# Zelana-Labs/zelana

Hardware: AMD Instinct MI355X
Metric: BN254 G1 MSM Mpoint-scalar/s + L2 proofs/sec at 1/2/4/8 MI355X (higher is better)
Workload: dtype u32

## Files before the change

### include/zkmi.h

```cpp
#ifndef ZKMI_H
#define ZKMI_H
#include <stddef.h>
#include <stdint.h>

#ifdef __cplusplus
extern "C" {
#endif

#define ZKMI_OK 0
#define ZKMI_EINVAL (-1)
#define ZKMI_ENODEV (-2)
#define ZKMI_EHIP (-3)
#define ZKMI_ENOMEM (-4)
#define ZKMI_EPOINT (-5)

typedef struct zkmi_ctx zkmi_ctx;
typedef struct zkmi_bases zkmi_bases;
typedef struct zkmi_pk zkmi_pk;
typedef struct zkmi_msm_job zkmi_msm_job;
typedef struct zkmi_r1cs_dev zkmi_r1cs_dev;

const char* zkmi_last_error(void);
int zkmi_version(void);

int zkmi_ctx_create(int device, zkmi_ctx** out);
void zkmi_ctx_destroy(zkmi_ctx* ctx);
int zkmi_profile_enable(zkmi_ctx* ctx, int on);
int zkmi_profile_get(zkmi_ctx* ctx, const char* name, double* total_ms, uint64_t* count);
int zkmi_profile_reset(zkmi_ctx* ctx);
int zkmi_dev_alloc(zkmi_ctx* ctx, size_t bytes, void** dptr);
int zkmi_dev_free(zkmi_ctx* ctx, void* dptr);
int zkmi_h2d(zkmi_ctx* ctx, void* dst, const void* src, size_t bytes);
int zkmi_d2h(zkmi_ctx* ctx, void* dst, const void* src, size_t bytes);
int zkmi_sync(zkmi_ctx* ctx);

int zkmi_bases_create_g1(zkmi_ctx* ctx, const uint64_t* affine, size_t n, zkmi_bases** out);
int zkmi_bases_create_g2(zkmi_ctx* ctx, const uint64_t* affine, size_t n, zkmi_bases** out);
void zkmi_bases_destroy(zkmi_bases* b);
size_t zkmi_bases_len(const zkmi_bases* b);
int zkmi_bases_export(const zkmi_bases* b, uint64_t* affine_out);
int zkmi_bases_precompute(zkmi_bases* b, int c, int factor);
int zkmi_bases_info(const zkmi_bases* b, uint64_t out[4]);
int zkmi_bases_generate_g1(zkmi_ctx* ctx, uint64_t seed, size_t n, zkmi_bases** out);
int zkmi_bases_generate_g2(zkmi_ctx* ctx, uint64_t seed, size_t n, zkmi_bases** out);
int zkmi_scalars_generate(zkmi_ctx* ctx, uint64_t seed, size_t n, void* d_scalars);
int zkmi_bases_generate_range_g1(zkmi_ctx* ctx, uint64_t seed, size_t first, size_t n, zkmi_bases** out);
int zkmi_scalars_generate_range(zkmi_ctx* ctx, uint64_t seed, size_t first, size_t n, void* d_scalars);
int zkmi_bases_generate_arith_g1(zkmi_ctx* ctx, const uint64_t p0[8], const uint64_t d[8], size_t first, size_t n,
                                 zkmi_bases** out);

int zkmi_msm_g1(zkmi_ctx* ctx, const zkmi_bases* b, size_t offset, const uint64_t* scalars, size_t n,
                uint64_t out_affine[8]);
int zkmi_msm_g2(zkmi_ctx* ctx, const zkmi_bases* b, size_t offset, const uint64_t* scalars, size_t n,
                uint64_t out_affine[16]);
int zkmi_msm_g1_device(zkmi_ctx* ctx, const zkmi_bases* b, size_t offset, const void* d_scalars, size_t n,
                       uint64_t out_affine[8]);
int zkmi_msm_g2_device(zkmi_ctx* ctx, const zkmi_bases* b, size_t offset, const void* d_scalars, size_t n,
                       uint64_t out_affine[16]);
int zkmi_msm_submit(zkmi_ctx* ctx, const zkmi_bases* b, size_t offset, const void* d_scalars, size_t n,
                    zkmi_msm_job** job);
int zkmi_msm_wait(zkmi_msm_job* job, uint64_t* out_affine);
int zkmi_msm_submit_shared(zkmi_ctx* ctx, const zkmi_bases* const* bs, int k, size_t offset, const void* d_scalars,
// ... 202 lines not shown
```

### zelana_amd/_lib.py

```python
from __future__ import annotations

import ctypes
import os

HERE = os.path.dirname(os.path.abspath(__file__))
LIB_PATH = os.environ.get("ZKMI_LIB") or os.path.join(HERE, "libzkmi.so")


class ZkmiError(RuntimeError):
    pass


_lib = None
vp = ctypes.c_void_p
u64p = ctypes.POINTER(ctypes.c_uint64)
u8p = ctypes.POINTER(ctypes.c_uint8)
sz = ctypes.c_size_t


class WprogDesc(ctypes.Structure):
    _fields_ = [
        ("num_vars", sz), ("num_inputs", sz), ("input_var", vp), ("num_ops", sz), ("op", vp),
        ("num_terms", sz), ("term", vp), ("num_coeffs", sz), ("coeff", vp), ("num_levels", sz),
        ("level_start", vp),
    ]


class R1CSStruct(ctypes.Structure):
    _fields_ = [
        ("num_constraints", sz), ("num_instance", sz), ("num_witness", sz),
        ("a_rowptr", vp), ("a_col", vp), ("a_val", vp),
        ("b_rowptr", vp), ("b_col", vp), ("b_val", vp),
        ("c_rowptr", vp), ("c_col", vp), ("c_val", vp),
    ]


class R1CSStatusStruct(ctypes.Structure):
    _fields_ = [("first_row", ctypes.c_uint64), ("n_bad", ctypes.c_uint64), ("a", ctypes.c_uint64 * 4),
                ("b", ctypes.c_uint64 * 4), ("c", ctypes.c_uint64 * 4)]


ROW_NONE = 2**64 - 1


class VerifyStatsStruct(ctypes.Structure):
    _fields_ = [("pairs", ctypes.c_uint64), ("final_exps", ctypes.c_uint64), ("invalid_points", ctypes.c_uint64)]


SIGNATURES = [
    ("zkmi_last_error", ctypes.c_char_p, []),
    ("zkmi_version", ctypes.c_int, []),
    ("zkmi_ctx_create", ctypes.c_int, [ctypes.c_int, ctypes.POINTER(vp)]),
    ("zkmi_ctx_destroy", None, [vp]),
    ("zkmi_profile_enable", ctypes.c_int, [vp, ctypes.c_int]),
    ("zkmi_profile_get", ctypes.c_int, [vp, ctypes.c_char_p, ctypes.POINTER(ctypes.c_double),
                                        ctypes.POINTER(ctypes.c_uint64)]),
    ("zkmi_profile_reset", ctypes.c_int, [vp]),
    ("zkmi_dev_alloc", ctypes.c_int, [vp, sz, ctypes.POINTER(vp)]),
    ("zkmi_dev_free", ctypes.c_int, [vp, vp]),
    ("zkmi_h2d", ctypes.c_int, [vp, vp, vp, sz]),
    ("zkmi_d2h", ctypes.c_int, [vp, vp, vp, sz]),
    ("zkmi_sync", ctypes.c_int, [vp]),
    ("zkmi_bases_create_g1", ctypes.c_int, [vp, u64p, sz, ctypes.POINTER(vp)]),
    ("zkmi_bases_create_g2", ctypes.c_int, [vp, u64p, sz, ctypes.POINTER(vp)]),
    ("zkmi_bases_destroy", None, [vp]),
    ("zkmi_bases_len", sz, [vp]),
    ("zkmi_bases_export", ctypes.c_int, [vp, u64p]),
    ("zkmi_bases_precompute", ctypes.c_int, [vp, ctypes.c_int, ctypes.c_int]),
    ("zkmi_bases_info", ctypes.c_int, [vp, u64p]),
    ("zkmi_bases_generate_g1", ctypes.c_int, [vp, ctypes.c_uint64, sz, ctypes.POINTER(vp)]),
    ("zkmi_bases_generate_g2", ctypes.c_int, [vp, ctypes.c_uint64, sz, ctypes.POINTER(vp)]),
    ("zkmi_scalars_generate", ctypes.c_int, [vp, ctypes.c_uint64, sz, vp]),
    ("zkmi_bases_generate_range_g1", ctypes.c_int, [vp, ctypes.c_uint64, sz, sz, ctypes.POINTER(vp)]),
    ("zkmi_bases_generate_arith_g1", ctypes.c_int, [vp, u64p, u64p, sz, sz, ctypes.POINTER(vp)]),
    ("zkmi_scalars_generate_range", ctypes.c_int, [vp, ctypes.c_uint64, sz, sz, vp]),
    ("zkmi_msm_g1", ctypes.c_int, [vp, vp, sz, u64p, sz, u64p]),
    ("zkmi_msm_g2", ctypes.c_int, [vp, vp, sz, u64p, sz, u64p]),
    ("zkmi_msm_g1_device", ctypes.c_int, [vp, vp, sz, vp, sz, u64p]),
    ("zkmi_msm_g2_device", ctypes.c_int, [vp, vp, sz, vp, sz, u64p]),
    ("zkmi_msm_submit", ctypes.c_int, [vp, vp, sz, vp, sz, ctypes.POINTER(vp)]),
    ("zkmi_msm_wait", ctypes.c_int, [vp, u64p]),
    ("zkmi_msm_set_window", ctypes.c_int, [vp, ctypes.c_int]),
    ("zkmi_msm_batch_submit", ctypes.c_int, [vp, vp, sz, vp, sz, sz, sz, ctypes.POINTER(vp)]),
    ("zkmi_msm_batch_wait", ctypes.c_int, [vp, u64p, sz]),
    ("zkmi_ctx_set_batch_group", ctypes.c_int, [vp, ctypes.c_int]),
    ("zkmi_ctx_get_batch_group", ctypes.c_int, [vp]),
    ("zkmi_msm_set_lanes", ctypes.c_int, [vp, ctypes.c_int]),
    ("zkmi_msm_get_lanes", ctypes.c_int, [vp]),
    ("zkmi_ctx_stream_count", ctypes.c_int, [vp]),
    ("zkmi_msm_submit_shared", ctypes.c_int, [vp, ctypes.POINTER(vp), ctypes.c_int, sz, vp, sz, ctypes.POINTER(vp)]),
# ... 129 lines not shown
```

### zelana_amd/csrc/ec.h

```cpp
#pragma once
#include "ff.h"

#if defined(__HIPCC__) || defined(__HIP__)
#define ZK_HD_NOINLINE __host__ __device__ __noinline__
#else
#define ZK_HD_NOINLINE inline
#endif

namespace zk {


template <class F>
struct Aff {
  typename F::T x, y;
};
template <class F>
struct Xyzz {
  typename F::T x, y, zz, zzz;
};

template <class F>
ZK_HD Xyzz<F> xyzz_inf() {
  Xyzz<F> r;
  r.x = F::zero();
// ... 93 lines not shown
  Fe qx = subk<FqP, 8>(qq, r.x);
  r.y = mul2<FqP>(rr, qx, ny1, ppp);
  r.zz = mul<FqP>(p.zz, pp);
  r.zzz = mul<FqP>(p.zzz, ppp);
  return r;
}
ZK_HD Xyzz<FqOps> xyzz_madd_g1f(const Xyzz<FqOps>& p, const Fe& qx, const Fe& qy, bool* inf) {
  const Fe ny1 = bsub(FqP::B4_1, p.y);
  const Fe pp_ = mul_add<FqP>(qx, p.zz, bsub(FqP::B8_1, p.x));
  const Fe rr = mul_add<FqP>(qy, p.zzz, ny1);
  const Fe pp = sqr<FqP>(pp_);
  uint32_t z = 0, e = 0;
#pragma unroll
  for (int i = 0; i < NL; i++) {
    z |= pp.v[i];
    e |= pp.v[i] ^ FqP::P[i];
  }
  *inf = false;
  if (z == 0 || e == 0) {
    if (is_zero<FqP>(reduce_q32<FqP>(rr))) return xyzz_mdbl(Aff<FqOps>{qx, reduce_q32<FqP>(qy)});
    *inf = true;
    return xyzz_inf<FqOps>();
  }
  const Fe ppp = mul<FqP>(pp_, pp);
  const Fe qq = mul<FqP>(p.x, pp);
  Xyzz<FqOps> r;
  r.x = sqr_add<FqP>(rr, bsub2(FqP::B6_3, ppp, qq));
  r.y = mul2<FqP>(rr, bsubadd(FqP::B10_1, r.x, qq), ny1, ppp);
  r.zz = mul<FqP>(p.zz, pp);
  r.zzz = mul<FqP>(p.zzz, ppp);
  return r;
}

ZK_HD Xyzz<FqOps> xyzz_mmadd_g1(const Aff<FqOps>& p, const Aff<FqOps>& q) {
  Fe pp_ = subk<FqP, 2>(q.x, p.x);
  Fe ny1 = subk<FqP, 2>(fe_zero(), p.y);
  Fe rr = add_lazy(q.y, ny1);
  Fe pp = sqr<FqP>(pp_);
  if (is_zero<FqP>(pp)) {
    Fe rn = reduce8<FqP>(subk<FqP, 2>(q.y, p.y));
    if (is_zero<FqP>(rn)) return xyzz_mdbl(q);
    return xyzz_inf<FqOps>();
  }
  Fe ppp = mul<FqP>(pp_, pp);
  Fe qq = mul<FqP>(p.x, pp);
  Fe t = add_lazy(add_lazy(ppp, qq), qq);
  Xyzz<FqOps> r;
  r.x = subk<FqP, 6>(sqr<FqP>(rr), t);
  Fe qx = subk<FqP, 8>(qq, r.x);
  r.y = mul2<FqP>(rr, qx, ny1, ppp);
  r.zz = pp;
  r.zzz = ppp;
  return r;
}
ZK_HD Xyzz<Fq2Ops> xyzz_mmadd_g2(const Aff<Fq2Ops>& p, const Aff<Fq2Ops>& q) {
  Fe2 pp_ = {subk<FqPn, 2>(q.x.c0, p.x.c0), subk<FqPn, 2>(q.x.c1, p.x.c1)};
  Fe2 rr = {subk<FqPn, 2>(q.y.c0, p.y.c0), subk<FqPn, 2>(q.y.c1, p.y.c1)};
  Fe2 pp = f2_sqr_n(pp_);
  if (f2_is_zero(pp)) {
    if (is_zero<FqPn>(reduce8<FqPn>(rr.c0)) && is_zero<FqPn>(reduce8<FqPn>(rr.c1))) return xyzz_mdbl(q);
    return xyzz_inf<Fq2Ops>();
  }
  Fe2 r2 = f2_sqr_n(rr);
  Fe2 ppp = f2_mul_n(pp_, pp), qq = f2_mul_n(p.x, pp);
  Xyzz<Fq2Ops> r;
  r.x.c0 = reduce8<FqPn>(subk<FqPn, 6>(r2.c0, add_lazy(add_lazy(ppp.c0, qq.c0), qq.c0)));
  r.x.c1 = reduce8<FqPn>(subk<FqPn, 6>(r2.c1, add_lazy(add_lazy(ppp.c1, qq.c1), qq.c1)));
  Fe2 qx = {subk<FqPn, 2>(qq.c0, r.x.c0), subk<FqPn, 2>(qq.c1, r.x.c1)};
  Fe ny0 = subk<FqPn, 2>(fe_zero(), p.y.c0), ny1 = subk<FqPn, 2>(fe_zero(), p.y.c1);
  Fe nqx1 = subk<FqPn, 4>(fe_zero(), qx.c1), nppp1 = subk<FqPn, 2>(fe_zero(), ppp.c1);
  r.y.c0 = mul4<FqPn>(rr.c0, qx.c0, rr.c1, nqx1, ny0, ppp.c0, ny1, nppp1);
  r.y.c1 = mul4<FqPn>(rr.c0, qx.c1, rr.c1, qx.c0, ny0, ppp.c1, ny1, ppp.c0);
  r.zz = pp;
  r.zzz = ppp;
  return r;
}
// ... 125 lines not shown
```

### zelana_amd/csrc/msm.hip

```cpp
#include <stdarg.h>
#include <stdlib.h>
#include <stdio.h>
#include <string.h>

#include <algorithm>
#include <string>
#include <type_traits>
#include <utility>
#include <vector>
#include <chrono>

#include "dev_io.h"
#include "ec.h"
#include "zkmi_internal.h"

namespace zk {

#define ZK_TAIL_WAVE() __builtin_amdgcn_s_setprio(3)

struct G1T {
  using F = FqOps;
  using P = FqP;
  static constexpr int CW = 8;
  static constexpr int PW = 16;
// ... 1059 lines not shown
#define ZK_ACC0_G2_MINBLK 2
#endif
#ifndef ZK_ACC0_G1_MINBLK
#define ZK_ACC0_G1_MINBLK 1
#endif
__global__ void __launch_bounds__(256, ZK_ACC0_G1_MINBLK) k_msm_acc0_g1(const uint32_t* __restrict__ sval, const uint32_t* __restrict__ bstart,
                                                  uint32_t K, uint32_t L, uint32_t nchunks,
                                                  const uint32_t* __restrict__ bases, uint32_t tn, uint32_t tskip,
                                                  uint32_t* __restrict__ buckets,
                                                  uint32_t* __restrict__ xkey, uint32_t* __restrict__ xvalid,
                                                  uint32_t* __restrict__ xpts, uint32_t* __restrict__ flags) { msm_acc0_body<G1T>(sval, bstart, K, L, nchunks, bases, tn, tskip, buckets, xkey, xvalid, xpts, flags); }
__global__ void __launch_bounds__(256, ZK_ACC0_G2_MINBLK) k_msm_acc0_g2(const uint32_t* __restrict__ sval, const uint32_t* __restrict__ bstart,
                                                  uint32_t K, uint32_t L, uint32_t nchunks,
                                                  const uint32_t* __restrict__ bases, uint32_t tn, uint32_t tskip,
                                                  uint32_t* __restrict__ buckets,
                                                  uint32_t* __restrict__ xkey, uint32_t* __restrict__ xvalid,
                                                  uint32_t* __restrict__ xpts, uint32_t* __restrict__ flags) { msm_acc0_body<G2T>(sval, bstart, K, L, nchunks, bases, tn, tskip, buckets, xkey, xvalid, xpts, flags); }
template <class G>
struct Acc0Kernel;
template <>
struct Acc0Kernel<G1T> {
  static constexpr auto fn = k_msm_acc0_g1;
};
template <>
struct Acc0Kernel<G2T> {
  static constexpr auto fn = k_msm_acc0_g2;
};

constexpr uint32_t ITEM_CAP_MAX = 1024;
constexpr uint32_t ITEMS_MIN_K = 1u << 18;
constexpr uint32_t NOSLOT = 0xFFFFFFFFu;

__device__ __forceinline__ bool item_of(const uint4* __restrict__ items, uint32_t nover, uint32_t nmain, uint32_t i,
                                        uint4& it) {
  uint32_t idx;
  if (i < nover) {
    idx = nmain + i;
  } else {
    idx = i - nover;
    if (idx >= nmain) return false;
  }
  it = items[idx];
  return it.x != it.y;
}

template <class G>
__device__ __forceinline__ void acc_items_body(const uint4* __restrict__ items, const uint32_t* __restrict__ nover,
                                               uint32_t nmain, const uint32_t* __restrict__ sval,
                                               const uint32_t* __restrict__ bases, uint32_t tn, uint32_t tskip,
                                               uint32_t* __restrict__ buckets, uint32_t* __restrict__ xpts) {
  using F = typename G::F;
  constexpr int XW = 4 * G::CW;
  constexpr int PQ = G::PW / 4;
  uint4 it;
  if (!item_of(items, *nover, nmain, blockIdx.x * blockDim.x + threadIdx.x, it)) return;
  const uint32_t start = it.x, end = it.y;
  auto row = [&](uint32_t v) {
    uint32_t idx = v & 0x7FFFFFFFu;
    if (tskip) idx += (idx / tn) * tskip;
    const uint32_t* src = bases;
    return reinterpret_cast<const uint4*>(src + (size_t)idx * G::PW);
  };
  constexpr bool PF = G::CW == 8;
  Xyzz<F> acc = xyzz_inf<F>();
  bool naff = false;
  uint32_t v_nxt = sval[start];
  uint4 raw[PQ];
  if constexpr (PF) {
    const uint4* q = row(v_nxt);
#pragma unroll
    for (int k = 0; k < PQ; k++) raw[k] = q[k];
  }
  uint32_t v_nn = start + 1 < end ? sval[start + 1] : 0u;
  for (uint32_t p = start; p < end; p++) {
    uint4 cr[PQ];
    const uint32_t v = v_nxt;
    if constexpr (PF) {
#pragma unroll
      for (int k = 0; k < PQ; k++) cr[k] = raw[k];
      if (p + 1 < end) {
        const uint4* q = row(v_nn);
#pragma unroll
        for (int k = 0; k < PQ; k++) raw[k] = q[k];
      }
    } else {
      const uint4* q = row(v);
#pragma unroll
      for (int k = 0; k < PQ; k++) cr[k] = q[k];
    }
    v_nxt = v_nn;
    if (p + 2 < end) v_nn = sval[p + 2];
    const uint32_t* w = reinterpret_cast<const uint32_t*>(cr);
    const bool binf = (w[G::PW - 1] >> 31) != 0;
    Aff<F> P;
    const bool ng = (v >> 31) != 0;
    if constexpr (G::CW == 8) {
      P.x = unpack(w);
      P.y = unpack(w + 8);
      if (ng) P.y = fq_cneg(P.y, true);
    } else {
      P.x = {unpack(w), unpack(w + 8)};
      P.y = {unpack(w + 16), unpack(w + 24)};
      if (ng) P.y = {fq_cneg(P.y.c0, true), fq_cneg(P.y.c1, true)};
    }
    const int mode = binf ? 3 : xyzz_is_inf(acc) ? 0 : (naff) ? 1 : 2;
    if (mode == 0) {
      acc = xyzz_from_aff(P);
      naff = true;
    } else if (mode == 1) {
      if constexpr (G::CW == 8) acc = xyzz_mmadd_g1({acc.x, acc.y}, P);
      else acc = xyzz_mmadd_g2({acc.x, acc.y}, P);
      naff = false;
    } else if (mode == 2) {
      if constexpr (G::CW == 8) acc = xyzz_madd_g1(acc, P);
      else acc = xyzz_madd_g2(acc, P);
    }
  }
  st_acc<G>(it.w == NOSLOT ? buckets + (size_t)it.z * XW : xpts + (size_t)it.w * XW, acc);
}
__device__ __forceinline__ void ld_row4(uint4 (&r)[4], const uint4* q) {
#pragma unroll
  for (int k = 0; k < 4; k++) r[k] = q[k];
}
__device__ __forceinline__ void acc_items_g1f(const uint4* __restrict__ items, const uint32_t* __restrict__ nover,
                                              uint32_t nmain, const uint32_t* __restrict__ sval,
                                              const uint32_t* __restrict__ bases, uint32_t tn, uint32_t tskip,
                                              uint32_t* __restrict__ buckets, uint32_t* __restrict__ xpts,
                                              uint32_t i) {
  using F = FqOps;
  constexpr int XW = 32;
  uint4 it;
  if (!item_of(items, *nover, nmain, i, it)) return;
  const uint32_t start = it.x, end = it.y;
  auto row = [&](uint32_t v) {
    uint32_t idx = v & 0x7FFFFFFFu;
    if (tskip) idx += (idx / tn) * tskip;
    const uint32_t* src = bases;
    return reinterpret_cast<const uint4*>(src + (size_t)idx * G1T::PW);
  };
  Xyzz<F> acc = xyzz_inf<F>();
  int phase = 0;
  auto step = [&](const uint4 (&r)[4], uint32_t v) {
    const uint32_t* w = reinterpret_cast<const uint32_t*>(r);
    const int mode = (w[G1T::PW - 1] >> 31) ? 3 : phase;
    const Fe x2 = unpack(w);
    const Fe y0 = unpack(w + 8);
    const Fe yn = bsub(FqP::B2_1, y0);
    const bool ng = (v >> 31) != 0;
    Fe y2;
#pragma unroll
    for (int k = 0; k < NL; k++) y2.v[k] = ng ? yn.v[k] : y0.v[k];
    if (mode == 2) {
      bool inf;
      acc = xyzz_madd_g1f(acc, x2, y2, &inf);
      if (inf) phase = 0;
    } else if (mode == 1) {
      acc = xyzz_mmadd_g1({acc.x, acc.y}, Aff<F>{x2, reduce_q32<FqP>(y2)});
      phase = xyzz_is_inf(acc) ? 0 : 2;
    } else if (mode == 0) {
      acc = xyzz_from_aff(Aff<F>{x2, reduce_q32<FqP>(y2)});
      phase = 1;
    }
  };
  uint4 raw[4];
  const uint32_t last = end - 1;
  uint32_t v_nxt = sval[start];
  ld_row4(raw, row(v_nxt));
  uint32_t v_nn = sval[min(start + 1, last)];
  for (uint32_t p = start; p < end; p++) {
    uint4 cr[4];
    const uint32_t v = v_nxt;
#pragma unroll
    for (int k = 0; k < 4; k++) cr[k] = raw[k];
    ld_row4(raw, row(v_nn));
    v_nxt = v_nn;
    v_nn = sval[min(p + 2, last)];
    step(cr, v);
  }
  if (phase == 0) acc = xyzz_inf<F>();
  st_acc<G1T>(it.w == NOSLOT ? buckets + (size_t)it.z * XW : xpts + (size_t)it.w * XW, acc);
}
template <bool VPAD>
__global__ void __launch_bounds__(256, ZK_ACC0_G1_MINBLK)
    k_acc_items_g1(const uint4* __restrict__ items, const uint32_t* __restrict__ nover, uint32_t nmain,
                   const uint32_t* __restrict__ sval, const uint32_t* __restrict__ bases, uint32_t tn,
                   uint32_t tskip, uint32_t* __restrict__ buckets, uint32_t* __restrict__ xpts) {
  if constexpr (VPAD) asm volatile("" ::: "v135");
  acc_items_g1f(items, nover, nmain, sval, bases, tn, tskip, buckets, xpts, blockIdx.x * blockDim.x + threadIdx.x);
}
__global__ void __launch_bounds__(256, ZK_ACC0_G2_MINBLK)
    k_acc_items_g2(const uint4* __restrict__ items, const uint32_t* __restrict__ nover, uint32_t nmain,
                   const uint32_t* __restrict__ sval, const uint32_t* __restrict__ bases, uint32_t tn,
                   uint32_t tskip, uint32_t* __restrict__ buckets, uint32_t* __restrict__ xpts) {
  acc_items_body<G2T>(items, nover, nmain, sval, bases, tn, tskip, buckets, xpts);
}

__global__ void __launch_bounds__(256) k_items_place(const uint4* __restrict__ stage, uint32_t NLO, uint32_t cap,
                                                     const uint32_t* __restrict__ ghist, uint32_t* __restrict__ gcur,
                                                     uint4* __restrict__ items, uint32_t nmain) {
  ZK_TAIL_WAVE();
  __shared__ uint32_t lh[ITEM_CAP_MAX + 1], lstart[ITEM_CAP_MAX + 1], base[ITEM_CAP_MAX + 1], tmp[4];
  const uint32_t h = blockIdx.x;
  const uint4* st = stage + (size_t)h * NLO;
  for (uint32_t c = threadIdx.x; c <= cap; c += 256) lh[c] = 0;
  __syncthreads();
  for (uint32_t x = threadIdx.x; x < NLO; x += 256) {
    const uint4 it = st[x];
    atomicAdd(&lh[min(it.y - it.x, cap)], 1u);
  }
  __syncthreads();
  block_prefix<256>(cap + 1, [&](uint32_t k) { return lh[cap - k]; }, lstart, tmp);
  block_prefix<256>(cap + 1, [&](uint32_t k) { return ghist[cap - k]; }, base, tmp);
  for (uint32_t k = threadIdx.x; k <= cap; k += 256) {
    const uint32_t c = cap - k;
    if (lh[c]) base[k] += atomicAdd(&gcur[c], lh[c]);
  }
  __syncthreads();
  for (uint32_t x = threadIdx.x; x < NLO; x += 256) {
    const uint4 it = st[x];
    const uint32_t k = cap - min(it.y - it.x, cap);
    const uint32_t dst = base[k] + (x - lstart[k]);
    if (dst < nmain) items[dst] = it;
  }
}

template <class G, bool CHUNKED = false>
__global__ void __launch_bounds__(256) k_split_combine(const uint4* __restrict__ split,
                                                       const uint32_t* __restrict__ nsplit,
                                                       const uint32_t* __restrict__ xpts,
                                                       uint32_t* __restrict__ buckets) {
  ZK_TAIL_WAVE();
  using F = typename G::F;
  constexpr int XW = 4 * G::CW;
  constexpr uint32_t BIG = 256;
  __shared__ Xyzz<F> sh[4][32];
  __shared__ uint4 spl[4];
  const uint32_t ns = *nsplit;
  const uint32_t wave = threadIdx.x >> 6, lane = threadIdx.x & 63;
  for (uint32_t base = blockIdx.x * 4; base < ns; base += gridDim.x * 4) {
    if (lane == 0) spl[wave] = base + wave < ns ? split[base + wave] : make_uint4(0, 0, 0, 0);
    __syncthreads();
    uint32_t mxs = 0;
    for (int w = 0; w < 4; w++) mxs = max(mxs, spl[w].z <= BIG ? spl[w].z : 0u);
    const uint32_t nload0 = (mxs + 63) / 64;
    uint32_t lev0 = 0;
    while ((1u << lev0) < min(mxs, 64u)) lev0++;
    const uint4 mine = spl[wave];
    const bool small = mine.z <= BIG;
    Xyzz<F> v = xyzz_inf<F>();
    int ph = 0;
    uint32_t st0 = 0;
    uint32_t nload = nload0, lev = lev0, cross = 0, stride = 64;
    uint4 cur = mine;
    bool mine_in = small;
    for (uint32_t step = 0;; step++) {
      uint32_t k = step - st0;
      if (k >= nload + lev + cross) {
        if (ph == 0) {
          if (small && mine.z && lane == 0) st_xyzz<G>(buckets + (size_t)mine.x * XW, v);
        } else if (threadIdx.x == 0) {
          st_xyzz<G>(buckets + (size_t)cur.x * XW, v);
        }
        v = xyzz_inf<F>();
        int w = ph;
        while (w < 4 && spl[w].z <= BIG) w++;
        if (w >= 4) break;
        ph = w + 1;
        cur = spl[w];
        mine_in = true;
// ... 1251 lines not shown
    ZK_TRY(comm_allgather_device(job->comm, st, d_buf, gathered, SHARD_PAYLOAD_WORDS * 4));
    job->exchanged = true;
    job->host_words = width;
    ZK_TRY(ctx_pinned_get(ctx, (size_t)nr * width * 4, (void**)&job->host));
    job->st = st;
    ZK_HIP(hipMemcpy2DAsync(job->host, width * 4, gathered, SHARD_PAYLOAD_WORDS * 4, width * 4, nr,
                            hipMemcpyDeviceToHost, st));
  } else {
    job->host_words = SHARD_PAYLOAD_WORDS;
    ZK_TRY(ctx_pinned_get(ctx, SHARD_PAYLOAD_WORDS * 4, (void**)&job->host));
    job->st = st;
    ZK_HIP(hipMemcpyAsync(job->host, d_buf, width * 4, hipMemcpyDeviceToHost, st));
  }
  ZK_HIP(hipEventRecord(job->done, st));
  job->done_rec = true;
  return 0;
}

template <class G>
static int msm_acc_phase(zkmi_ctx* ctx, MsmLane* lane, const MsmPlan& P, const zkmi_bases* tb, size_t offset,
                         size_t n, const uint32_t* sval, const uint32_t* bstart, zkmi_msm_job* job) {
  constexpr int XW = 4 * G::CW;
  using GS = std::conditional_t<G::CW == 8, G1Tn, G>;
  using GB = G;
  hipStream_t st = lane->st;
  Workspace& ws = lane->ws;
  const uint32_t* d_bases = tb->d_pts + offset * G::PW;
  const uint32_t K = P.K;
  const int W = P.W, bb = P.bb, lb = P.lb, hb = P.hb;
  const size_t Mmax = P.Mmax;
  const uint32_t tn = (uint32_t)n, tskip = P.p > 1 ? (uint32_t)(tb->n - n) : 0u;
  uint32_t* buckets;
  ZK_TRY(ws.get("msm_buckets", (size_t)K * XW * 4, (void**)&buckets));
  if (items_plan(P)) {
    const BsGeom g = bs_geom(P, n);
    const uint32_t cap = item_cap(ctx, P);
    const size_t npieces = (Mmax + cap - 1) / cap;
    const size_t items_max = g.nmain + npieces;
    uint32_t* ctr = lane->bs_cur;
    uint32_t* xpts;
    uint4 *items, *split;
    ZK_TRY(ws.get("msm_items", items_max * 16, (void**)&items));
    ZK_TRY(ws.get("msm_split", (npieces + 1) * 16, (void**)&split));
    ZK_TRY(ws.get("msm_xpts", (2 * npieces + 2) * XW * 4, (void**)&xpts));
    const uint32_t* itc = ctr + g.NH;
    if (ctx->acc_last && ctx->acc_last != lane) ZK_HIP(hipStreamWaitEvent(st, ctx->acc_last->acc_done, 0));
    {
      ScopedKernelTimer tm(ctx, G::CW == 8 ? "msm_acc0_g1" : "msm_acc0_g2", st);
#ifndef ZK_ACC_VPAD_LOG
#define ZK_ACC_VPAD_LOG 27
#endif
      const bool vpad = G::CW == 8 && Mmax >= ((size_t)1 << std::min(ZK_ACC_VPAD_LOG, 63));
      auto kern = G::CW == 8 ? (vpad ? k_acc_items_g1<true> : k_acc_items_g1<false>) : k_acc_items_g2;
#ifndef ZK_ACC_LDS_B
#define ZK_ACC_LDS_B 41984
#endif
      const size_t acc_lds = G::CW == 8 && !vpad ? (size_t)ZK_ACC_LDS_B : 0;
      kern<<<(unsigned)((items_max + 255) / 256), 256, acc_lds, st>>>(
          items, &itc[0], (uint32_t)g.nmain, sval, d_bases, tn, tskip, buckets, xpts);
    }
    ZK_HIP(hipEventRecord(lane->acc_done, st));
    ctx->acc_last = lane;
    ScopedKernelTimer tm(ctx, "msm_accN", st);
    auto comb = K <= CUTSUM_COOP_K ? k_split_combine<GS> : k_split_combine<GB>;
    const size_t maxsplit = std::min<size_t>(K, npieces / 2 + 1);
    comb<<<(unsigned)std::min<size_t>((maxsplit + 3) / 4, 1024), 256, 0, st>>>(split, &itc[2], xpts, buckets);
    ZK_HIP(hipGetLastError());
  } else {
    uint32_t *flags, *xkey, *xvalid, *xpts, *ykey, *yvalid, *ypts;
    ZK_TRY(ws.get("msm_flags", 64 * 4, (void**)&flags));
    const size_t tpc = 1024;
    const size_t acc_threads = (size_t)ctx->num_cus * tpc;
    uint32_t L = (uint32_t)std::max<size_t>(4, (Mmax + acc_threads - 1) / acc_threads);
    uint32_t nch = (uint32_t)((Mmax + L - 1) / L);
    const size_t xl = 2 * (size_t)nch + 1;
    ZK_TRY(ws.get("msm_xkey", xl * 4 + 64, (void**)&xkey));
    ZK_TRY(ws.get("msm_xvalid", xl * 4 + 64, (void**)&xvalid));
    ZK_TRY(ws.get("msm_xpts", (xl + 2) * XW * 4, (void**)&xpts));
    ZK_TRY(ws.get("msm_ykey", xl * 4 + 64, (void**)&ykey));
    ZK_TRY(ws.get("msm_yvalid", xl * 4 + 64, (void**)&yvalid));
    ZK_TRY(ws.get("msm_ypts", (xl + 2) * XW * 4, (void**)&ypts));
    {
      ScopedKernelTimer tm(ctx, G::CW == 8 ? "msm_acc0_g1" : "msm_acc0_g2", st);
      Acc0Kernel<G>::fn<<<(nch + 255) / 256, 256, 0, st>>>(sval, bstart, K, L, nch, d_bases, tn, tskip, buckets, xkey,
                                                            xvalid, xpts, flags);
      ZK_HIP(hipGetLastError());
    }
    ScopedKernelTimer tm(ctx, "msm_accN", st);
#ifndef ZK_SMALL_SPLIT
#define ZK_SMALL_SPLIT 1
#endif
    if (ZK_SMALL_SPLIT && K <= CUTSUM_COOP_K) {
      const size_t maxsplit = std::min<size_t>(K, nch / 16 + 1);
      uint4* split;
      ZK_TRY(ws.get("msm_small_split", maxsplit * 16, (void**)&split));
      k_msm_cutsum_coop<GS><<<(unsigned)(((size_t)K * 16 + 255) / 256), 256, 0, st>>>(bstart, K, L, buckets, xvalid,
                                                                                   xpts, &flags[0], split, &flags[32]);
      k_split_combine<GS, true><<<(unsigned)std::min<size_t>((maxsplit + 3) / 4, 256), 256, 0, st>>>(split, &flags[32],
                                                                                                  xpts, buckets);
// ... 482 lines not shown
```

### zelana_amd/csrc/zkmi_api.hip

```cpp
#include <stdarg.h>
#include <stdio.h>
#include <string.h>

#include <algorithm>

#include <atomic>

#include "zkmi_internal.h"

namespace zk {

static thread_local char g_err[512] = "";
void set_error(const char* fmt, ...) {
  va_list ap;
  va_start(ap, fmt);
  vsnprintf(g_err, sizeof(g_err), fmt, ap);
  va_end(ap);
}

void note_cleared_error(hipError_t e, const char* fn) {
  static std::atomic<int> seen{0};
  if (seen.fetch_add(1) < 8)
    fprintf(stderr, "libzkmi: %s entered with a pending HIP error (%s); cleared\n", fn ? fn : "?",
            hipGetErrorString(e));
// ... 151 lines not shown
    hipEventDestroy(l->consumed);
    hipEventDestroy(l->acc_done);
    hipStreamDestroy(l->st);
    delete l;
  }
  ctx->lanes.clear();
  ctx->nstreams = 1;
  if (ctx->prove_fork) hipEventDestroy(ctx->prove_fork);
  if (ctx->wm_done) hipEventDestroy(ctx->wm_done);
  for (auto& pb : ctx->pinned_free) hipHostFree(pb.first);
  ctx->pinned_free.clear();
  ctx->pinned_size.clear();
  hipStreamDestroy(ctx->stream);
  delete ctx;
}
int zkmi_profile_enable(zkmi_ctx* ctx, int on) {
  ctx->timer.enabled = on != 0;
  return 0;
}
int zkmi_profile_get(zkmi_ctx* ctx, const char* name, double* total_ms, uint64_t* count) {
  ZK_DEVICE_GUARD(ctx);
  ZK_TRY(timer_flush(ctx));
  auto it = ctx->timer.totals.find(name);
  *total_ms = it == ctx->timer.totals.end() ? 0.0 : it->second.first;
  *count = it == ctx->timer.totals.end() ? 0 : it->second.second;
  return 0;
}
int zkmi_profile_reset(zkmi_ctx* ctx) {
  ZK_DEVICE_GUARD(ctx);
  ZK_TRY(timer_flush(ctx));
  ctx->timer.totals.clear();
  return 0;
}
int zkmi_dev_alloc(zkmi_ctx* ctx, size_t bytes, void** dptr) {
  ZK_DEVICE_GUARD(ctx);
  if (hipMalloc(dptr, bytes ? bytes : 1) != hipSuccess) {
    (void)hipGetLastError();
    set_error("hipMalloc(%zu) failed", bytes);
    return ZKMI_ENOMEM;
  }
  return 0;
}
int zkmi_dev_free(zkmi_ctx* ctx, void* dptr) {
  ZK_DEVICE_GUARD(ctx);
  ZK_HIP(hipFree(dptr));
  return 0;
}
int zkmi_h2d(zkmi_ctx* ctx, void* dst, const void* src, size_t bytes) {
  ZK_DEVICE_GUARD(ctx);
  ZK_HIP(hipMemcpyAsync(dst, src, bytes, hipMemcpyHostToDevice, ctx->stream));
  ZK_HIP(hipStreamSynchronize(ctx->stream));
  return 0;
}
int zkmi_d2h(zkmi_ctx* ctx, void* dst, const void* src, size_t bytes) {
  ZK_DEVICE_GUARD(ctx);
  ZK_HIP(hipMemcpyAsync(dst, src, bytes, hipMemcpyDeviceToHost, ctx->stream));
  ZK_HIP(hipStreamSynchronize(ctx->stream));
  return 0;
}
int zkmi_sync(zkmi_ctx* ctx) {
  ZK_DEVICE_GUARD(ctx);
  return ctx_sync_all(ctx);
}

int zkmi_bases_create_g1(zkmi_ctx* ctx, const uint64_t* affine, size_t n, zkmi_bases** out) {
  ZK_DEVICE_GUARD(ctx);
// ... 232 lines not shown
```

### zelana_amd/csrc/zkmi_internal.h

```cpp
#pragma once
#include <hip/hip_runtime.h>
#include <stdint.h>

#include <map>
#include <string>
#include <vector>

#include "../../include/zkmi.h"
#include "zkmi_internal_host.h"

namespace zk {

void set_error(const char* fmt, ...);

#define ZK_HIP(expr)                                                                       \
  do {                                                                                     \
    hipError_t e_ = (expr);                                                                \
    if (e_ != hipSuccess) {                                                                \
      ::zk::set_error("HIP error %s at %s:%d (%s)", hipGetErrorString(e_), __FILE__, __LINE__, #expr); \
      return ZKMI_EHIP;                                                                    \
    }                                                                                      \
  } while (0)

#define ZK_TRY(expr)          \
// ... 21 lines not shown
  bool bs_dirty = false;
  void* ss_clean = nullptr;
  size_t ss_clean_words = 0;
  uint32_t* bs_cur = nullptr;
};

struct KernelTimer {
  bool enabled = false;
  struct Rec {
    hipEvent_t a, b;
    std::string name;
  };
  std::vector<Rec> pending;
  std::map<std::string, std::pair<double, uint64_t>> totals;
};

}

struct zkmi_ctx {
  int device = 0;
  hipStream_t stream = nullptr;
  zk::Workspace ws;
  std::vector<std::pair<void*, size_t>> pinned_free;
  std::map<void*, size_t> pinned_size;
  zk::KernelTimer timer;
  int msm_window = 0;
  int num_cus = 256;
  int msm_lanes = 2;
  int batch_group = 0;
  int lane_next = 0;
  std::vector<zk::MsmLane*> lanes;
  hipEvent_t msm_fork = nullptr;
  zk::MsmLane* acc_last = nullptr;
  hipEvent_t prove_fork = nullptr;
  hipEvent_t acc_gate = nullptr;
  const zkmi_bases* acc_gate_set = nullptr;
  hipEvent_t wm_done = nullptr;
  int prove_check = 0;
  std::vector<zkmi_r1cs_status> last_check;
  uint64_t verify_probes = 0;
  uint64_t verify_last[3] = {0, 0, 0};
  int ncomm = 0;
  int nstreams = 0;
  std::vector<zkmi_wprog*> wprogs;
};
constexpr int MAX_LANES_WITH_COMM = 2;

struct zkmi_bases {
  zkmi_ctx* ctx;
  int g2;
  size_t n;
  uint32_t* d_pts;
  int tc = 0;
  int tp = 1;
  int tw = 0;
  int tbal = 0;
};

constexpr int ZKMI_COMM_RCCL = 0;
constexpr int ZKMI_COMM_HOST = 1;
struct zkmi_comm {
  zkmi_ctx* ctx = nullptr;
  uint64_t serial = 0;
  int nranks = 1, rank = 0, kind = ZKMI_COMM_RCCL;
  void* nccl = nullptr;
  hipStream_t st = nullptr;
// ... 99 lines not shown
```

### zelana_amd/gpu.py

```python
from __future__ import annotations

import ctypes
import weakref
from dataclasses import dataclass

import numpy as np

from ._lib import ROW_NONE, R1CSStatusStruct, R1CSStruct, VerifyStatsStruct, ZkmiError, check, lib, u64p, u8p, vp


def _p64(a: np.ndarray):
    assert a.dtype == np.uint64 and a.flags.c_contiguous
    return a.ctypes.data_as(u64p)


class DeviceBuffer:
    def __init__(self, ctx: "Context", nbytes: int):
        self.ctx, self.nbytes = ctx, nbytes
        self.ptr = vp()
        check(lib().zkmi_dev_alloc(ctx.h, nbytes, ctypes.byref(self.ptr)), "zkmi_dev_alloc")

    def upload(self, arr: np.ndarray):
        arr = np.ascontiguousarray(arr)
        assert arr.nbytes <= self.nbytes
# ... 84 lines not shown
        self._deps = weakref.WeakSet()
        check(lib().zkmi_ctx_create(device, ctypes.byref(self.h)), "zkmi_ctx_create")

    def _track(self, obj):
        self._deps.add(obj)
        return obj

    def close(self):
        if self.h:
            for obj in list(self._deps):
                try:
                    obj.close()
                except Exception:
                    pass
            lib().zkmi_ctx_destroy(self.h)
            self.h = vp()

    def __del__(self):
        try:
            self.close()
        except Exception:
            pass

    def profile(self, on: bool = True):
        check(lib().zkmi_profile_enable(self.h, int(on)))

    def profile_get(self, name: str):
        t, c = ctypes.c_double(), ctypes.c_uint64()
        check(lib().zkmi_profile_get(self.h, name.encode(), ctypes.byref(t), ctypes.byref(c)))
        return t.value, c.value

    def profile_reset(self):
        check(lib().zkmi_profile_reset(self.h))

    def set_window(self, c: int):
        check(lib().zkmi_msm_set_window(self.h, c))

    def set_batch_group(self, g: int):
        check(lib().zkmi_ctx_set_batch_group(self.h, g), "zkmi_ctx_set_batch_group")

    def batch_group(self) -> int:
        return lib().zkmi_ctx_get_batch_group(self.h)

    def set_prove_check(self, on: bool):
        check(lib().zkmi_ctx_set_prove_check(self.h, int(bool(on))), "zkmi_ctx_set_prove_check")

    def prove_check(self) -> bool:
        return lib().zkmi_ctx_get_prove_check(self.h) == 1

    def set_verify_probes(self, n: int):
        check(lib().zkmi_ctx_set_verify_probes(self.h, int(n)), "zkmi_ctx_set_verify_probes")

    def get_verify_probes(self) -> int:
        return int(lib().zkmi_ctx_get_verify_probes(self.h))

    def set_lanes(self, lanes: int):
        check(lib().zkmi_msm_set_lanes(self.h, lanes))

    def lanes(self) -> int:
        return lib().zkmi_msm_get_lanes(self.h)

    def stream_count(self) -> int:
        return lib().zkmi_ctx_stream_count(self.h)

    def sync(self):
        check(lib().zkmi_sync(self.h))
# ... 818 lines not shown
```

Before: 973.5.

## Use unchecked G1 bucket adds with a deferred exact redo pass for degenerate items

The G1 bucket accumulation kernel now uses mixed and affine addition formulas that skip the per-step checks for doubling and infinity. It instead detects a poisoned result (ZZ equal to zero or p) at the end and appends that item's index to a redo list. A new tail kernel reprocesses those rare items with the exact, branchy accumulator, and the split-combine kernel resets the redo counter. This removes branches and reductions from the hot loop in exchange for an extra kernel launch, an atomic per degenerate item, and a dependence on degeneracies being rare and correctly detected.

```diff
diff --git a/include/zkmi.h b/include/zkmi.h
--- a/include/zkmi.h
+++ b/include/zkmi.h
@@ -28,6 +28,7 @@
 int zkmi_profile_enable(zkmi_ctx* ctx, int on);
 int zkmi_profile_get(zkmi_ctx* ctx, const char* name, double* total_ms, uint64_t* count);
 int zkmi_profile_reset(zkmi_ctx* ctx);
+int zkmi_msm_last_redo(zkmi_ctx* ctx, uint64_t* count);
 int zkmi_dev_alloc(zkmi_ctx* ctx, size_t bytes, void** dptr);
 int zkmi_dev_free(zkmi_ctx* ctx, void* dptr);
 int zkmi_h2d(zkmi_ctx* ctx, void* dst, const void* src, size_t bytes);
diff --git a/zelana_amd/_lib.py b/zelana_amd/_lib.py
--- a/zelana_amd/_lib.py
+++ b/zelana_amd/_lib.py
@@ -56,6 +56,7 @@
     ("zkmi_profile_get", ctypes.c_int, [vp, ctypes.c_char_p, ctypes.POINTER(ctypes.c_double),
                                         ctypes.POINTER(ctypes.c_uint64)]),
     ("zkmi_profile_reset", ctypes.c_int, [vp]),
+    ("zkmi_msm_last_redo", ctypes.c_int, [vp, u64p]),
     ("zkmi_dev_alloc", ctypes.c_int, [vp, sz, ctypes.POINTER(vp)]),
     ("zkmi_dev_free", ctypes.c_int, [vp, vp]),
     ("zkmi_h2d", ctypes.c_int, [vp, vp, vp, sz]),
diff --git a/zelana_amd/csrc/ec.h b/zelana_amd/csrc/ec.h
--- a/zelana_amd/csrc/ec.h
+++ b/zelana_amd/csrc/ec.h
@@ -149,6 +149,30 @@
   return r;
 }
 
+ZK_HD Xyzz<FqOps> xyzz_madd_g1u(const Xyzz<FqOps>& p, const Fe& qx, const Fe& qy) {
+  const Fe ny1 = bsub(FqP::B4_1, p.y);
+  const Fe pp_ = mul_add<FqP>(qx, p.zz, bsub(FqP::B8_1, p.x));
+  const Fe rr = mul_add<FqP>(qy, p.zzz, ny1);
+  const Fe pp = sqr<FqP>(pp_);
+  const Fe ppp = mul<FqP>(pp_, pp);
+  const Fe qq = mul<FqP>(p.x, pp);
+  Xyzz<FqOps> r;
+  r.x = sqr_add<FqP>(rr, bsub2(FqP::B6_3, ppp, qq));
+  r.y = mul2<FqP>(rr, bsubadd(FqP::B10_1, r.x, qq), ny1, ppp);
+  r.zz = mul<FqP>(p.zz, pp);
+  r.zzz = mul<FqP>(p.zzz, ppp);
+  return r;
+}
+ZK_HD bool xyzz_g1u_poisoned(const Xyzz<FqOps>& p) {
+  uint32_t z = 0, e = 0;
+#pragma unroll
+  for (int i = 0; i < NL; i++) {
+    z |= p.zz.v[i];
+    e |= p.zz.v[i] ^ FqP::P[i];
+  }
+  return z == 0 || e == 0;
+}
+
 ZK_HD Xyzz<FqOps> xyzz_mmadd_g1(const Aff<FqOps>& p, const Aff<FqOps>& q) {
   Fe pp_ = subk<FqP, 2>(q.x, p.x);
   Fe ny1 = subk<FqP, 2>(fe_zero(), p.y);
@@ -159,6 +183,22 @@
     if (is_zero<FqP>(rn)) return xyzz_mdbl(q);
     return xyzz_inf<FqOps>();
   }
+  Fe ppp = mul<FqP>(pp_, pp);
+  Fe qq = mul<FqP>(p.x, pp);
+  Fe t = add_lazy(add_lazy(ppp, qq), qq);
+  Xyzz<FqOps> r;
+  r.x = subk<FqP, 6>(sqr<FqP>(rr), t);
+  Fe qx = subk<FqP, 8>(qq, r.x);
+  r.y = mul2<FqP>(rr, qx, ny1, ppp);
+  r.zz = pp;
+  r.zzz = ppp;
+  return r;
+}
+ZK_HD Xyzz<FqOps> xyzz_mmadd_g1u(const Aff<FqOps>& p, const Aff<FqOps>& q) {
+  Fe pp_ = subk<FqP, 2>(q.x, p.x);
+  Fe ny1 = subk<FqP, 2>(fe_zero(), p.y);
+  Fe rr = add_lazy(q.y, ny1);
+  Fe pp = sqr<FqP>(pp_);
   Fe ppp = mul<FqP>(pp_, pp);
   Fe qq = mul<FqP>(p.x, pp);
   Fe t = add_lazy(add_lazy(ppp, qq), qq);
diff --git a/zelana_amd/csrc/msm.hip b/zelana_amd/csrc/msm.hip
--- a/zelana_amd/csrc/msm.hip
+++ b/zelana_amd/csrc/msm.hip
@@ -1115,8 +1115,7 @@
 constexpr uint32_t NOSLOT = 0xFFFFFFFFu;
 
 __device__ __forceinline__ bool item_of(const uint4* __restrict__ items, uint32_t nover, uint32_t nmain, uint32_t i,
-                                        uint4& it) {
-  uint32_t idx;
+                                        uint4& it, uint32_t& idx) {
   if (i < nover) {
     idx = nmain + i;
   } else {
@@ -1126,17 +1125,19 @@
   it = items[idx];
   return it.x != it.y;
 }
+__device__ __forceinline__ bool item_of(const uint4* __restrict__ items, uint32_t nover, uint32_t nmain, uint32_t i,
+                                        uint4& it) {
+  uint32_t idx;
+  return item_of(items, nover, nmain, i, it, idx);
+}
 
 template <class G>
-__device__ __forceinline__ void acc_items_body(const uint4* __restrict__ items, const uint32_t* __restrict__ nover,
-                                               uint32_t nmain, const uint32_t* __restrict__ sval,
+__device__ __forceinline__ void acc_item_exact(const uint4 it, const uint32_t* __restrict__ sval,
                                                const uint32_t* __restrict__ bases, uint32_t tn, uint32_t tskip,
                                                uint32_t* __restrict__ buckets, uint32_t* __restrict__ xpts) {
   using F = typename G::F;
   constexpr int XW = 4 * G::CW;
   constexpr int PQ = G::PW / 4;
-  uint4 it;
-  if (!item_of(items, *nover, nmain, blockIdx.x * blockDim.x + threadIdx.x, it)) return;
   const uint32_t start = it.x, end = it.y;
   auto row = [&](uint32_t v) {
     uint32_t idx = v & 0x7FFFFFFFu;
@@ -1201,6 +1202,15 @@
   }
   st_acc<G>(it.w == NOSLOT ? buckets + (size_t)it.z * XW : xpts + (size_t)it.w * XW, acc);
 }
+template <class G>
+__device__ __forceinline__ void acc_items_body(const uint4* __restrict__ items, const uint32_t* __restrict__ nover,
+                                               uint32_t nmain, const uint32_t* __restrict__ sval,
+                                               const uint32_t* __restrict__ bases, uint32_t tn, uint32_t tskip,
+                                               uint32_t* __restrict__ buckets, uint32_t* __restrict__ xpts) {
+  uint4 it;
+  if (!item_of(items, *nover, nmain, blockIdx.x * blockDim.x + threadIdx.x, it)) return;
+  acc_item_exact<G>(it, sval, bases, tn, tskip, buckets, xpts);
+}
 __device__ __forceinline__ void ld_row4(uint4 (&r)[4], const uint4* q) {
 #pragma unroll
   for (int k = 0; k < 4; k++) r[k] = q[k];
@@ -1209,7 +1219,8 @@
                                               uint32_t nmain, const uint32_t* __restrict__ sval,
                                               const uint32_t* __restrict__ bases, uint32_t tn, uint32_t tskip,
                                               uint32_t* __restrict__ buckets, uint32_t* __restrict__ xpts,
-                                              uint32_t i) {
+                                              uint32_t* __restrict__ nredo, uint32_t* __restrict__ redo,
+                                              uint32_t rcap, uint32_t i) {
   using F = FqOps;
   constexpr int XW = 32;
   uint4 it;
@@ -1234,12 +1245,10 @@
 #pragma unroll
     for (int k = 0; k < NL; k++) y2.v[k] = ng ? yn.v[k] : y0.v[k];
     if (mode == 2) {
-      bool inf;
-      acc = xyzz_madd_g1f(acc, x2, y2, &inf);
-      if (inf) phase = 0;
+      acc = xyzz_madd_g1u(acc, x2, y2);
     } else if (mode == 1) {
-      acc = xyzz_mmadd_g1({acc.x, acc.y}, Aff<F>{x2, reduce_q32<FqP>(y2)});
-      phase = xyzz_is_inf(acc) ? 0 : 2;
+      acc = xyzz_mmadd_g1u({acc.x, acc.y}, Aff<F>{x2, reduce_q32<FqP>(y2)});
+      phase = 2;
     } else if (mode == 0) {
       acc = xyzz_from_aff(Aff<F>{x2, reduce_q32<FqP>(y2)});
       phase = 1;
@@ -1260,16 +1269,35 @@
     v_nn = sval[min(p + 2, last)];
     step(cr, v);
   }
-  if (phase == 0) acc = xyzz_inf<F>();
+  if (phase == 2 && xyzz_g1u_poisoned(acc)) {
+    const uint32_t no = *nover, k = atomicAdd(nredo, 1u);
+    if (k < rcap) redo[k] = i < no ? nmain + i : i - no;
+    return;
+  }
   st_acc<G1T>(it.w == NOSLOT ? buckets + (size_t)it.z * XW : xpts + (size_t)it.w * XW, acc);
 }
 template <bool VPAD>
 __global__ void __launch_bounds__(256, ZK_ACC0_G1_MINBLK)
     k_acc_items_g1(const uint4* __restrict__ items, const uint32_t* __restrict__ nover, uint32_t nmain,
                    const uint32_t* __restrict__ sval, const uint32_t* __restrict__ bases, uint32_t tn,
-                   uint32_t tskip, uint32_t* __restrict__ buckets, uint32_t* __restrict__ xpts) {
+                   uint32_t tskip, uint32_t* __restrict__ buckets, uint32_t* __restrict__ xpts,
+                   uint32_t* __restrict__ nredo, uint32_t* __restrict__ redo, uint32_t rcap) {
   if constexpr (VPAD) asm volatile("" ::: "v135");
-  acc_items_g1f(items, nover, nmain, sval, bases, tn, tskip, buckets, xpts, blockIdx.x * blockDim.x + threadIdx.x);
+  acc_items_g1f(items, nover, nmain, sval, bases, tn, tskip, buckets, xpts, nredo, redo, rcap,
+                blockIdx.x * blockDim.x + threadIdx.x);
+}
+__global__ void __launch_bounds__(256)
+    k_acc_redo_g1(const uint4* __restrict__ items, const uint32_t* __restrict__ nredo,
+                  const uint32_t* __restrict__ redo, uint32_t rcap, const uint32_t* __restrict__ sval,
+                  const uint32_t* __restrict__ bases, uint32_t tn, uint32_t tskip, uint32_t* __restrict__ buckets,
+                  uint32_t* __restrict__ xpts, uint32_t* __restrict__ last) {
+  ZK_TAIL_WAVE();
+  const uint32_t n = min(*nredo, rcap);
+  if (last && blockIdx.x == 0 && threadIdx.x == 0) *last = n;
+  for (uint32_t k = blockIdx.x * 256 + threadIdx.x; k < n; k += gridDim.x * 256) {
+    const uint32_t idx = redo[k];
+    if (idx < rcap) acc_item_exact<G1T>(items[idx], sval, bases, tn, tskip, buckets, xpts);
+  }
 }
 __global__ void __launch_bounds__(256, ZK_ACC0_G2_MINBLK)
     k_acc_items_g2(const uint4* __restrict__ items, const uint32_t* __restrict__ nover, uint32_t nmain,
@@ -1311,13 +1339,15 @@
 __global__ void __launch_bounds__(256) k_split_combine(const uint4* __restrict__ split,
                                                        const uint32_t* __restrict__ nsplit,
                                                        const uint32_t* __restrict__ xpts,
-                                                       uint32_t* __restrict__ buckets) {
+                                                       uint32_t* __restrict__ buckets,
+                                                       uint32_t* __restrict__ clr = nullptr) {
   ZK_TAIL_WAVE();
   using F = typename G::F;
   constexpr int XW = 4 * G::CW;
   constexpr uint32_t BIG = 256;
   __shared__ Xyzz<F> sh[4][32];
   __shared__ uint4 spl[4];
+  if (clr && blockIdx.x == 0 && threadIdx.x == 0) *clr = 0;
   const uint32_t ns = *nsplit;
   const uint32_t wave = threadIdx.x >> 6, lane = threadIdx.x & 63;
   for (uint32_t base = blockIdx.x * 4; base < ns; base += gridDim.x * 4) {
@@ -2635,6 +2665,7 @@
   const uint32_t tn = (uint32_t)n, tskip = P.p > 1 ? (uint32_t)(tb->n - n) : 0u;
   uint32_t* buckets;
   ZK_TRY(ws.get("msm_buckets", (size_t)K * XW * 4, (void**)&buckets));
+  ctx->redo_last_set = false;
   if (items_plan(P)) {
     const BsGeom g = bs_geom(P, n);
     const uint32_t cap = item_cap(ctx, P);
@@ -2646,7 +2677,14 @@
     ZK_TRY(ws.get("msm_items", items_max * 16, (void**)&items));
     ZK_TRY(ws.get("msm_split", (npieces + 1) * 16, (void**)&split));
     ZK_TRY(ws.get("msm_xpts", (2 * npieces + 2) * XW * 4, (void**)&xpts));
-    const uint32_t* itc = ctr + g.NH;
+    uint32_t* itc = ctr + g.NH;
+    uint32_t *redo = nullptr, *redo_last = nullptr;
+    if (G::CW == 8) ZK_TRY(ws.get("msm_redo", items_max * 4, (void**)&redo));
+    if (G::CW == 8 && ctx->timer.enabled) {
+      ZK_TRY(ctx->ws.get("msm_redo_last", 4, (void**)&redo_last));
+      ctx->redo_last = redo_last;
+      ctx->redo_last_set = true;
+    }
     if (ctx->acc_last && ctx->acc_last != lane) ZK_HIP(hipStreamWaitEvent(st, ctx->acc_last->acc_done, 0));
     {
       ScopedKernelTimer tm(ctx, G::CW == 8 ? "msm_acc0_g1" : "msm_acc0_g2", st);
@@ -2654,20 +2692,31 @@
 #define ZK_ACC_VPAD_LOG 27
 #endif
       const bool vpad = G::CW == 8 && Mmax >= ((size_t)1 << std::min(ZK_ACC_VPAD_LOG, 63));
-      auto kern = G::CW == 8 ? (vpad ? k_acc_items_g1<true> : k_acc_items_g1<false>) : k_acc_items_g2;
 #ifndef ZK_ACC_LDS_B
 #define ZK_ACC_LDS_B 41984
 #endif
       const size_t acc_lds = G::CW == 8 && !vpad ? (size_t)ZK_ACC_LDS_B : 0;
-      kern<<<(unsigned)((items_max + 255) / 256), 256, acc_lds, st>>>(
-          items, &itc[0], (uint32_t)g.nmain, sval, d_bases, tn, tskip, buckets, xpts);
+      const unsigned grid = (unsigned)((items_max + 255) / 256);
+      if constexpr (G::CW == 8)
+        (vpad ? k_acc_items_g1<true> : k_acc_items_g1<false>)<<<grid, 256, acc_lds, st>>>(
+            items, &itc[0], (uint32_t)g.nmain, sval, d_bases, tn, tskip, buckets, xpts, &itc[3], redo,
+            (uint32_t)items_max);
+      else
+        k_acc_items_g2<<<grid, 256, acc_lds, st>>>(items, &itc[0], (uint32_t)g.nmain, sval, d_bases, tn, tskip,
+                                                   buckets, xpts);
     }
     ZK_HIP(hipEventRecord(lane->acc_done, st));
     ctx->acc_last = lane;
+    if constexpr (G::CW == 8) {
+      ScopedKernelTimer tm(ctx, "msm_acc_redo", st);
+      k_acc_redo_g1<<<(unsigned)std::min<size_t>((items_max + 255) / 256, 256), 256, 0, st>>>(
+          items, &itc[3], redo, (uint32_t)items_max, sval, d_bases, tn, tskip, buckets, xpts, redo_last);
+    }
     ScopedKernelTimer tm(ctx, "msm_accN", st);
     auto comb = K <= CUTSUM_COOP_K ? k_split_combine<GS> : k_split_combine<GB>;
     const size_t maxsplit = std::min<size_t>(K, npieces / 2 + 1);
-    comb<<<(unsigned)std::min<size_t>((maxsplit + 3) / 4, 1024), 256, 0, st>>>(split, &itc[2], xpts, buckets);
+    comb<<<(unsigned)std::min<size_t>((maxsplit + 3) / 4, 1024), 256, 0, st>>>(split, &itc[2], xpts, buckets,
+                                                                               G::CW == 8 ? &itc[3] : nullptr);
     ZK_HIP(hipGetLastError());
   } else {
     uint32_t *flags, *xkey, *xvalid, *xpts, *ykey, *yvalid, *ypts;
diff --git a/zelana_amd/csrc/zkmi_api.hip b/zelana_amd/csrc/zkmi_api.hip
--- a/zelana_amd/csrc/zkmi_api.hip
+++ b/zelana_amd/csrc/zkmi_api.hip
@@ -207,6 +207,16 @@
   ctx->timer.totals.clear();
   return 0;
 }
+int zkmi_msm_last_redo(zkmi_ctx* ctx, uint64_t* count) {
+  ZK_DEVICE_GUARD(ctx);
+  *count = 0;
+  if (!ctx->redo_last_set) return 0;
+  ZK_TRY(ctx_sync_all(ctx));
+  uint32_t v = 0;
+  ZK_HIP(hipMemcpy(&v, ctx->redo_last, 4, hipMemcpyDeviceToHost));
+  *count = v;
+  return 0;
+}
 int zkmi_dev_alloc(zkmi_ctx* ctx, size_t bytes, void** dptr) {
   ZK_DEVICE_GUARD(ctx);
   if (hipMalloc(dptr, bytes ? bytes : 1) != hipSuccess) {
diff --git a/zelana_amd/csrc/zkmi_internal.h b/zelana_amd/csrc/zkmi_internal.h
--- a/zelana_amd/csrc/zkmi_internal.h
+++ b/zelana_amd/csrc/zkmi_internal.h
@@ -77,6 +77,8 @@
   std::vector<zk::MsmLane*> lanes;
   hipEvent_t msm_fork = nullptr;
   zk::MsmLane* acc_last = nullptr;
+  uint32_t* redo_last = nullptr;
+  bool redo_last_set = false;
   hipEvent_t prove_fork = nullptr;
   hipEvent_t acc_gate = nullptr;
   const zkmi_bases* acc_gate_set = nullptr;
diff --git a/zelana_amd/gpu.py b/zelana_amd/gpu.py
--- a/zelana_amd/gpu.py
+++ b/zelana_amd/gpu.py
@@ -140,6 +140,11 @@
 
     def profile_reset(self):
         check(lib().zkmi_profile_reset(self.h))
+
+    def msm_last_redo(self) -> int:
+        c = ctypes.c_uint64()
+        check(lib().zkmi_msm_last_redo(self.h, ctypes.byref(c)), "zkmi_msm_last_redo")
+        return c.value
 
     def set_window(self, c: int):
         check(lib().zkmi_msm_set_window(self.h, c))
```

New measurement: 973.6, median of 2. No clear change (+0.0%).
